# autonomousvision/transfuser

Measured on AMD Instinct MI355X. Metric: training samples/sec (RGB+LiDAR pair), bs=10/GPU, higher is better.
Workload: dtype f32; 1 GPU; TransFuser LidarCenterNet (RegNetY-3.2GF x2, 168.0 M params) full train step, B=10/GPU, 3x256x704 RGB + 3x256x256 BEV, fp32, dropout 0.10, hipGraph replay; global_batch=10, parallelism=dp1, grad_allreduce=none (1 rank), build_id=21d3d8ecc43e0770

## Files before the change

### include/transfuser_hip.h

```cpp
#ifndef TRANSFUSER_HIP_H
#define TRANSFUSER_HIP_H
#include <stdint.h>
#ifdef __cplusplus
extern "C" {
#endif

int tf_version(void);
const char* tf_last_error(void);
const char* tf_build_id(void);
long tf_streamk_launches(void);
int tf_gemm_epi16(int on);
long tf_gemm_epi16_launches(void);

int tf_set_precision(int mode);
int tf_get_precision(void);
int tf_autotune(int enable);
int tf_force_plan(int bm, int bn, int bk, int splitk);
int tf_force_dma(int kind, int splitk);
int tf_plans_count(void);
int tf_plans_clear(void);
int tf_plans_save(const char* path);
int tf_plans_load(const char* path);


// ... 14 lines not shown
int tf_gemm_f32(const tf_gemm_desc* d, void* stream);
long tf_gemm_splitk_ws_floats(const tf_gemm_desc* d);
int tf_gemm_pair_begin(void);
int tf_gemm_pair_end(void* stream);
long tf_gemm_pair_count(int singles);

typedef struct {
    int B, Hi, Wi, Cin, Ho, Wo, Cout, ksize, stride, pad, groups;
} tf_conv_geom;
int tf_conv2d_fwd_f32(const tf_conv_geom* g, const float* x, const float* w, const float* bias, float* y, int relu, void* stream);
int tf_conv2d_fwd_colstat_f32(const tf_conv_geom* g, const float* x, const float* w, const float* bias, float* y, float* colstat, int* colstat_nparts,
                              void* stream);
int tf_conv2d_dgrad_f32(const tf_conv_geom* g, const float* dy, const float* w, float* dx, int accumulate, void* stream);
int tf_conv2d_wgrad_f32(const tf_conv_geom* g, const float* dy, const float* x, float* dw, int accumulate, void* stream);

int tf_conv3x3_small_fwd_f32(const float* x, const float* w, const float* bias, float* y, int B, int H, int W, int Cin, int Cout, int relu, void* stream);
int tf_conv3x3_small_dgrad_f32(const float* dy, const float* w, float* dx, int B, int H, int W, int Cin, int Cout, int accumulate, void* stream);
long tf_conv3x3_small_wgrad_ws_floats(void);
int tf_conv3x3_small_wgrad_f32(const float* dy, const float* x, float* dw, int B, int H, int W, int Cin, int Cout, int accumulate, float* ws, void* stream);

int tf_bn_finalize_parts_f32(const float* parts, int nparts, int rows, int C, const float* gamma, const float* beta, float* running_mean, float* running_var,
                             float momentum, float eps, float* save_mean, float* save_invstd, float* coef_out, void* stream);
int tf_colsum_bnrelu_parts_f32(const float* x, const float* coef, int nseg, int rows_per_seg, int C, float* ws, int* nchunks, void* stream);
int tf_se_excite_fwd_parts_f32(const float* parts, int nchunks, float scale, const float* W1, const float* b1, const float* W2, const float* b2, int B, int C,
                               int Cr, float* s_out, float* g1, float* gate, float* bwd_scratch, void* stream);
int tf_se_scale_bn_fwd_f32(const float* x, const float* coef, const float* gate, float* y, int B, int HW, int C, void* stream);
int tf_se_gate_grad_parts_f32(const float* dy, const float* x, const float* coef, int B, int HW, int C, float* ws, int* nchunks, void* stream);
int tf_se_excite_bwd_parts_f32(const float* parts, int nchunks, const float* gate, const float* s, const float* g1, const float* W1, const float* W2, int B,
                               int C, int Cr, float* dW1, float* db1, float* dW2, float* db2, float* ds, float* scratch, int scratch_is_zero, void* stream);
int tf_bn_bwd_remask_f32(const float* dz, const float* x, const float* fwd_coef, int rows, int C, const float* gamma, const float* save_mean,
                         const float* save_invstd, float* dx, float* dgamma, float* dbeta, float* ws, void* stream);
int tf_bn_bwd_remask_se_f32(const float* dy, const float* gate, const float* dmean, int B, int HW, int C, const float* x, const float* fcoef, const float* gamma,
                            const float* save_mean, const float* save_invstd, float* dx, float* dgamma, float* dbeta, float* ws, void* stream);

int tf_dwconv7_fwd_f32(const float* x, const float* w, const float* bias, float* y, int B, int H, int W, int C, int flip, int accumulate, void* stream);
int tf_dwconv7_wgrad_f32(const float* dy, const float* x, float* dw, float* dbias, int B, int H, int W, int C, void* stream);
int tf_gelu_fwd_f32(const float* x, float* y, int64_t n, void* stream);
int tf_gelu_bwd_f32(const float* dy, const float* x, float* dx, int64_t n, void* stream);
int tf_colscale_add_f32(const float* x, const float* gamma, const float* beta, const float* res, float* y, int64_t rows, int C, void* stream);
int tf_colsum_mul_f32(const float* a, const float* b, int rows, int C, float* out, int accumulate, float* ws, void* stream);
int tf_colsum_multi_f32(int n, const float* const* xs, const int* Cs, const long* lds, float* const* outs, int rows, void* stream);

int tf_cast16_f32(const float* x, int rows, int cols, int ldx, void* y16, int ldy, void* y16t, int ldyt, int dtype, void* stream);
typedef struct { const float* x; void* y16; void* y16t; int rows, cols, ldx, ldy, ldyt, tile0; } tf_cast16_item;
int tf_cast16_multi_f32(const tf_cast16_item* items_dev, int n_items, int total_tiles, int dtype, void* stream);
int tf_bn_apply16_f32(const float* x, const float* coef, const float* res, int relu, float* y32, int rows, int C, void* y16, void* y16t, int ldyt, int dtype, void* stream);
int tf_se_scale_bn16_f32(const float* x, const float* coef, const float* gate, int B, int HW, int C, void* y16, void* y16t, int ldyt, int dtype, void* stream);
int tf_bn_bwd16_f32(const float* dz, const float* z, const float* x, int rows, int C, const float* gamma, const float* save_mean, const float* save_invstd, float* dx32,
                    float* dres, float* dgamma, float* dbeta, float* ws, void* dx16, void* dx16t, int ldyt, int dtype, void* stream);
int tf_bn_bwd_remask16_f32(const float* dz, const float* x, const float* fcoef, int rows, int C, const float* gamma, const float* save_mean, const float* save_invstd,
                           float* dx32, float* dgamma, float* dbeta, float* ws, void* dx16, void* dx16t, int ldyt, int dtype, void* stream);
int tf_layernorm_fwd16_f32(const float* x, const float* gamma, const float* beta, void* y16, int ldy, void* y16t, int ldyt, float* mean, float* rstd,
                           int rows, int C, float eps, int dtype, void* stream);
int tf_gemm16_nt_f32(const void* a16, const void* b16, float* c, int m, int n, int k, int lda, int ldb, int ldc, const float* bias, const float* res, int ldres,
                     float alpha, int relu, int accumulate, const float* mask, int ldmask, int dtype, void* stream);
int tf_gemm16_nt_colstat_f32(const void* a16, const void* b16, float* c, int m, int n, int k, int lda, int ldb, int ldc, int dtype, float* colstat,
                             int* colstat_nparts, void* stream);
int tf_add_strided2_f32(const float* src, float* dst, int B, int Ho, int Wo, int C, int Hi, int Wi, void* stream);
int tf_im2col3x3_f32(const float* x, float* cols, int B, int H, int W, int C, void* stream);

int tf_conv3x3_thin_supported(int Cin, int Cout);
int tf_conv3x3_thin_fwd_f32(const float* x, const float* w, const float* bias, float* y, int B, int H, int W, int Cin, int Cout, void* stream);
int tf_conv3x3_thin_dgrad_f32(const float* dy, const float* w, const float* relu_mask, float* dx, int B, int H, int W, int Cin, int Cout, int accumulate,
                              void* stream);
long tf_conv3x3_thin_wgrad_ws_floats(void);
int tf_conv3x3_thin_wgrad_f32(const float* dy, const float* x, float* dw, float* dbias, int B, int H, int W, int Cin, int Cout, int accumulate, float* ws,
// ... 171 lines not shown
```

### transfuser_amd/csrc/reduce.cpp

```cpp
#include <cstdlib>
#include "tf_common.h"
#include "../../include/transfuser_hip.h"

using namespace tf;

namespace {

template <int V> struct vecf { float v[V]; };
template <int V> __device__ __forceinline__ vecf<V> ldv(const float* p) {
    vecf<V> r;
    if (V == 4) { float4 t = *reinterpret_cast<const float4*>(p); r.v[0] = t.x; r.v[1 % V] = t.y; r.v[2 % V] = t.z; r.v[3 % V] = t.w; }
    else r.v[0] = *p;
    return r;
}
template <int V> __device__ __forceinline__ void stv(float* p, const vecf<V>& a) {
    if (V == 4) *reinterpret_cast<float4*>(p) = make_float4(a.v[0], a.v[1 % V], a.v[2 % V], a.v[3 % V]);
    else *p = a.v[0];
}

constexpr int kBnSlots = 16;
constexpr int kMaxChunks = 512;
constexpr long kWsFloats = 4L << 20;
constexpr int kTickets = 4096;

// ... 78 lines not shown
template <int V> struct BnReluMulF {
    const float* dy; const float* x; const float* coef; int C;
    __device__ __forceinline__ void eval(long row, int c, vecf<V>* o) const {
        vecf<V> g = ldv<V>(dy + row * C + c), a = ldv<V>(x + row * C + c), sc = ldv<V>(coef + c), sh = ldv<V>(coef + C + c);
#pragma unroll
        for (int i = 0; i < V; ++i) o[0].v[i] = g.v[i] * fmaxf(a.v[i] * sc.v[i] + sh.v[i], 0.f);
    }
};
template <int V> struct BnBwdRemaskF {
    const float* dz; const float* x; const float* coef; const float* mean; const float* invstd; int C;
    __device__ __forceinline__ void eval(long row, int c, vecf<V>* o) const {
        vecf<V> g = ldv<V>(dz + row * C + c), a = ldv<V>(x + row * C + c), m = ldv<V>(mean + c), s = ldv<V>(invstd + c), sc = ldv<V>(coef + c), sh = ldv<V>(coef + C + c);
#pragma unroll
        for (int i = 0; i < V; ++i) {
            if (!(a.v[i] * sc.v[i] + sh.v[i] > 0.f)) g.v[i] = 0.f;
            o[0].v[i] = g.v[i];
            o[1].v[i] = g.v[i] * ((a.v[i] - m.v[i]) * s.v[i]);
        }
    }
};

template <int V> struct SeBnBwdRemaskF {
    const float* dy; const float* gate; const float* dmean; const float* x; const float* coef; const float* mean; const float* invstd; int C; int HW; float inv_hw;
    __device__ __forceinline__ void eval(long row, int c, vecf<V>* o) const {
        const long bc = (row / HW) * C + c;
        vecf<V> g = ldv<V>(dy + row * C + c), a = ldv<V>(x + row * C + c), m = ldv<V>(mean + c), s = ldv<V>(invstd + c), sc = ldv<V>(coef + c), sh = ldv<V>(coef + C + c);
        vecf<V> gt = ldv<V>(gate + bc), dm = ldv<V>(dmean + bc);
#pragma unroll
        for (int i = 0; i < V; ++i) {
            float gi = g.v[i] * (1.f / (1.f + expf(-gt.v[i]))) + dm.v[i] * inv_hw;
            if (!(a.v[i] * sc.v[i] + sh.v[i] > 0.f)) gi = 0.f;
            o[0].v[i] = gi;
            o[1].v[i] = gi * ((a.v[i] - m.v[i]) * s.v[i]);
        }
    }
};

template <int V, int NACC, class F>
__global__ void __launch_bounds__(256) colreduce_kernel(F f, int rows_per_seg, int C, int CTV, int rows_per_chunk, float* __restrict__ ws, int atomic,
                                                        float scale) {
    __shared__ __attribute__((aligned(16))) float red[NACC][256][V];
    const int tid = threadIdx.x;
    const int rpp = 256 / CTV;
    const int cq = tid % CTV, rl = tid / CTV;
    const int c = (blockIdx.x * CTV + cq) * V;
    const int seg = blockIdx.z, chunk = blockIdx.y;
    const int r0 = chunk * rows_per_chunk;
    int r1 = r0 + rows_per_chunk;
    if (r1 > rows_per_seg) r1 = rows_per_seg;
    vecf<V> acc[NACC];
#pragma unroll
    for (int a = 0; a < NACC; ++a)
#pragma unroll
        for (int i = 0; i < V; ++i) acc[a].v[i] = 0.f;
    if (rl < rpp) {
        const long base = (long)seg * rows_per_seg;
        int r = r0 + rl;
        if (atomic >= 0)
            for (; r < r1; r += 4 * rpp) {
                vecf<V> o[4][NACC];
#pragma unroll
                for (int u = 0; u < 4; ++u) {
                    const int rr = r + u * rpp;
                    f.eval(base + (rr < r1 ? rr : r1 - 1), c, o[u]);
                }
#pragma unroll
// ... 171 lines not shown
    coef[c] = sc;
    coef[C + c] = beta[c] - mean * sc;
    if (rmean) {
        rmean[c] = (1.f - momentum) * rmean[c] + momentum * mean;
        const float unb = (n > 1.f) ? var * (n / (n - 1.f)) : var;
        rvar[c] = (1.f - momentum) * rvar[c] + momentum * unb;
    }
}
__global__ void bn_eval_coef_kernel(const float* __restrict__ gamma, const float* __restrict__ beta, const float* __restrict__ rmean,
                                    const float* __restrict__ rvar, float* __restrict__ coef, int C, float eps) {
    const int c = blockIdx.x * 256 + threadIdx.x;
    if (c >= C) return;
    const float sc = gamma[c] / sqrtf(rvar[c] + eps);
    coef[c] = sc;
    coef[C + c] = beta[c] - rmean[c] * sc;
}
__global__ void __launch_bounds__(256) bn_bwd_finalize_kernel(const float* __restrict__ ws, const float* __restrict__ gamma, const float* __restrict__ mean,
                                                              const float* __restrict__ invstd, float* __restrict__ dgamma, float* __restrict__ dbeta,
                                                              float* __restrict__ coef, int C, int nch, float n) {
    const int c0 = blockIdx.x * 4 + (threadIdx.x >> 6), lane = threadIdx.x & 63;
    const bool live = c0 < C;
    const int c = live ? c0 : 0;
    float sg, sgx;
    chunk_sum2(ws + c, ws + C + c, 2L * C, nch, lane, live, sg, sgx);
    if (!live || lane != 0) return;
    if (dgamma) dgamma[c] += sgx;
    if (dbeta) dbeta[c] += sg;
    const float A = gamma[c] * invstd[c];
    const float Bc = -A * invstd[c] * (sgx / n);
    coef[c] = A;
    coef[C + c] = Bc;
    coef[2 * C + c] = -A * (sg / n) - Bc * mean[c];
}
__global__ void __launch_bounds__(256) se_bwd_finalize_kernel(const float* __restrict__ ws, const float* __restrict__ gate, float* __restrict__ dgate, int C,
                                                              int nch, int nseg) {
    const int i = blockIdx.x * 4 + (threadIdx.x >> 6), lane = threadIdx.x & 63;
    const bool live = i < nseg * C;
    const int seg = live ? i / C : 0, c = live ? i - seg * C : 0;
    const float s = chunk_sum(ws + (long)seg * nch * C + c, C, nch, lane, live);
    if (live && lane == 0) {
        const float sg = 1.f / (1.f + expf(-gate[i]));
        dgate[i] = s * sg * (1.f - sg);
    }
}

template <int V>
__global__ void __launch_bounds__(256) bn_apply_kernel(const float* __restrict__ x, const float* __restrict__ coef, const float* __restrict__ res,
                                                       float* __restrict__ y, long nvec, int C, int relu) {
    const int cv = C / V;
    for (long i = (long)blockIdx.x * 256 + threadIdx.x; i < nvec; i += (long)gridDim.x * 256) {
        const int c = (int)(i % cv) * V;
        vecf<V> a = ldv<V>(x + i * V), s = ldv<V>(coef + c), t = ldv<V>(coef + C + c);
        vecf<V> r;
        if (res) r = ldv<V>(res + i * V);
#pragma unroll
        for (int k = 0; k < V; ++k) {
            float v = a.v[k] * s.v[k] + t.v[k];
            if (res) v += r.v[k];
            if (relu) v = fmaxf(v, 0.f);
            a.v[k] = v;
        }
        stv<V>(y + i * V, a);
    }
}
template <int V>
__global__ void __launch_bounds__(256) bn_bwd_apply_kernel(const float* __restrict__ dz, const float* __restrict__ z, const float* __restrict__ x,
// ... 507 lines not shown
    const bool v4 = (C % 4 == 0) && aligned16(dz) && aligned16(x) && aligned16(dx) && aligned16(fcoef);
    RedPlan p = plan_reduce(rows, C, 1, 2, v4);
    BnBwdRemaskF<4> f4{dz, x, fcoef, save_mean, save_invstd, C};
    BnBwdRemaskF<1> f1{dz, x, fcoef, save_mean, save_invstd, C};
    launch_reduce<2>(p, f4, f1, rows, C, 1, ws, stream);
    TF_LAUNCH(bn_bwd_finalize_kernel, dim3(cdiv(C, 4)), dim3(256), stream, (const float*)ws, gamma, save_mean, save_invstd, dgamma, dbeta, coef, C, p.nchunks,
              (float)rows);
    const long n = (long)rows * C;
    if (v4) TF_LAUNCH(bn_bwd_apply_remask_kernel<4>, dim3(ew_blocks(n / 4)), dim3(256), stream, dz, x, fcoef, (const float*)coef, dx, n / 4, C);
    else TF_LAUNCH(bn_bwd_apply_remask_kernel<1>, dim3(ew_blocks(n)), dim3(256), stream, dz, x, fcoef, (const float*)coef, dx, n, C);
    return launch_status("tf_bn_bwd_remask_f32");
}

extern "C" int tf_bn_bwd_remask_se_f32(const float* dy, const float* gate, const float* dmean, int B, int HW, int C, const float* x, const float* fcoef,
                                       const float* gamma, const float* save_mean, const float* save_invstd, float* dx, float* dgamma, float* dbeta, float* ws,
                                       void* stream) {
    TF_REQUIRE(dy && gate && dmean && x && fcoef && gamma && save_mean && save_invstd && dx && ws && B > 0 && HW > 0 && C > 0, "tf_bn_bwd_remask_se_f32: bad arguments");
    const int rows = B * HW;
    float* coef = ws + kWsFloats / 2;
    const bool v4 = (C % 4 == 0) && aligned16(dy) && aligned16(x) && aligned16(dx) && aligned16(fcoef) && aligned16(gate) && aligned16(dmean);
    RedPlan p = plan_reduce(rows, C, 1, 2, v4);
    const float inv_hw = 1.f / (float)HW;
    SeBnBwdRemaskF<4> f4{dy, gate, dmean, x, fcoef, save_mean, save_invstd, C, HW, inv_hw};
    SeBnBwdRemaskF<1> f1{dy, gate, dmean, x, fcoef, save_mean, save_invstd, C, HW, inv_hw};
    launch_reduce<2>(p, f4, f1, rows, C, 1, ws, stream);
    TF_LAUNCH(bn_bwd_finalize_kernel, dim3(cdiv(C, 4)), dim3(256), stream, (const float*)ws, gamma, save_mean, save_invstd, dgamma, dbeta, coef, C, p.nchunks,
              (float)rows);
    const long n = (long)rows * C;
    if (v4) TF_LAUNCH(bn_bwd_apply_remask_se_kernel<4>, dim3(ew_blocks(n / 4)), dim3(256), stream, dy, gate, dmean, x, fcoef, (const float*)coef, dx, n / 4, C, (long)HW * C / 4, inv_hw);
    else TF_LAUNCH(bn_bwd_apply_remask_se_kernel<1>, dim3(ew_blocks(n)), dim3(256), stream, dy, gate, dmean, x, fcoef, (const float*)coef, dx, n, C, (long)HW * C, inv_hw);
    return launch_status("tf_bn_bwd_remask_se_f32");
}

extern "C" int tf_colsum_mul_f32(const float* a, const float* b, int rows, int C, float* out, int accumulate, float* ws, void* stream) {
    TF_REQUIRE(a && b && out && ws && rows > 0 && C > 0, "tf_colsum_mul_f32: bad arguments");
    RedPlan p = plan_reduce(rows, C, 1, 1, aligned16(a) && aligned16(b));
    MulF<4> f4{a, b, C};
    MulF<1> f1{a, b, C};
    launch_reduce<1>(p, f4, f1, rows, C, 1, ws, stream);
    TF_LAUNCH(colsum_finalize_kernel, dim3(cdiv((long)C, 4)), dim3(256), stream, (const float*)ws, out, C, p.nchunks, 1, 1.f, accumulate);
    return launch_status("tf_colsum_mul_f32");
}

extern "C" int tf_colsum_multi_f32(int n, const float* const* xs, const int* Cs, const long* lds, float* const* outs, int rows, void* stream) {
    TF_REQUIRE(n >= 1 && n <= kMultiMax && xs && Cs && lds && outs && rows > 0, "tf_colsum_multi_f32: 1 <= n <= %d matrices with rows > 0", kMultiMax);
    MultiSum d;
    d.n = n;
    int strips = 0;
    for (int i = 0; i < kMultiMax; ++i) {
        const int j = i < n ? i : n - 1;
        d.x[i] = xs[j]; d.out[i] = outs[j]; d.C[i] = Cs[j]; d.ld[i] = lds[j];
        d.strip0[i] = strips;
        if (i < n) {
            TF_REQUIRE(xs[i] && outs[i] && Cs[i] > 0 && Cs[i] % 4 == 0 && lds[i] % 4 == 0 && lds[i] >= Cs[i] && aligned16(xs[i]),
                       "tf_colsum_multi_f32: entry %d needs C %% 4 == 0, ld %% 4 == 0, ld >= C and a 16-byte aligned base", i);
            strips += cdiv(Cs[i], 32);
        }
    }
    d.strip0[kMultiMax] = strips;
    TF_LAUNCH(colsum_multi_kernel, dim3(strips), dim3(256), stream, d, rows);
    return launch_status("tf_colsum_multi_f32");
}

extern "C" int tf_bn_apply16_f32(const float* x, const float* coef, const float* res, int relu, float* y32, int rows, int C, void* y16, void* y16t, int ldyt,
                                 int dtype, void* stream) {
    TF_REQUIRE(x && coef && tile16_ok(rows, C, y16, y16t, ldyt, dtype) && aligned16(x) && aligned16(coef) && (!res || aligned16(res)) && (!y32 || aligned16(y32)),
// ... 44 lines not shown
```

### transfuser_amd/csrc/se.cpp

```cpp
#include "tf_common.h"
#include "../../include/transfuser_hip.h"

using namespace tf;

namespace {

constexpr int SE_MAXB = 16;
constexpr int SE_SPLIT = 8;
constexpr int SE_U = 4;
constexpr int SE_MAXC = 3072, SE_MAXR = 1024;

__device__ __forceinline__ float dot4(const float4 a, const float4 b) { return a.x * b.x + a.y * b.y + a.z * b.z + a.w * b.w; }

template <int U, int NK>
__device__ __forceinline__ void se_dots(const float* const* w, const float* __restrict__ vec, int n4, int lane, float* acc) {
    float4 wv[U][NK];
#pragma unroll
    for (int i = 0; i < NK; ++i) {
        const int k4 = lane + 64 * i, kc = k4 < n4 ? k4 : n4 - 1;
#pragma unroll
        for (int u = 0; u < U; ++u) wv[u][i] = reinterpret_cast<const float4*>(w[u])[kc];
    }
#pragma unroll
    for (int i = 0; i < NK; ++i) {
// ... 97 lines not shown
            }
        }
        __syncthreads();
        for (int nb = n0 + wave * SE_U; nb < n1; nb += nw * SE_U) {
            float acc[SE_U];
            const float* w[SE_U];
#pragma unroll
            for (int u = 0; u < SE_U; ++u) {
                acc[u] = 0.f;
                w[u] = W2 + (long)((nb + u < n1) ? nb + u : n1 - 1) * Cr;
            }
            for (int j = lane; j < Cr; j += 64) {
#pragma unroll
                for (int u = 0; u < SE_U; ++u) acc[u] += w[u][j] * hh[j];
            }
#pragma unroll
            for (int u = 0; u < SE_U; ++u) {
                const float a = wave_sum(acc[u]);
                if (lane == 0 && nb + u < n1) store2(nb + u, a);
            }
        }
    }
}

__global__ void __launch_bounds__(256) se_zero_kernel(float* __restrict__ p, int n) {
    const int i = blockIdx.x * 256 + threadIdx.x;
    if (i < n) p[i] = 0.f;
}

constexpr int SE_ROWS = 8;
__global__ void __launch_bounds__(256) se_excite_bwd2_kernel(const float* __restrict__ dgate, const float* __restrict__ g1, const float* __restrict__ W2,
                                                             int B, int C, int Cr, float* __restrict__ dW2, float* __restrict__ db2,
                                                             float* __restrict__ dg1, float* __restrict__ ds_zero, int nch = 0,
                                                             const float* __restrict__ gate = nullptr) {
    __shared__ float dgs[SE_MAXB][SE_ROWS];
    for (long i = (long)blockIdx.x * 256 + threadIdx.x; i < (long)B * C; i += (long)gridDim.x * 256) ds_zero[i] = 0.f;
    __shared__ float g1s[SE_MAXB * SE_MAXR / 2];
    const int n0 = blockIdx.x * SE_ROWS, tid = threadIdx.x;
    const int rows = (C - n0 < SE_ROWS) ? C - n0 : SE_ROWS;
    for (int i = tid; i < B * SE_ROWS; i += 256) {
        const int b = i / SE_ROWS, r = i % SE_ROWS;
        float v = 0.f;
        if (r < rows) {
            if (nch > 0) {
                const float* p = dgate + (long)b * nch * C + n0 + r;
                float v1 = 0.f, v2 = 0.f, v3 = 0.f;
                int j = 0;
                for (; j + 3 < nch; j += 4) { v += p[(long)j * C]; v1 += p[(long)(j + 1) * C]; v2 += p[(long)(j + 2) * C]; v3 += p[(long)(j + 3) * C]; }
                for (; j < nch; ++j) v += p[(long)j * C];
                v = (v + v1) + (v2 + v3);
                const float sg = 1.f / (1.f + expf(-gate[(long)b * C + n0 + r]));
                v *= sg * (1.f - sg);
            } else {
                v = dgate[(long)b * C + n0 + r];
            }
        }
        dgs[b][r] = v;
    }
    for (int i = tid; i < B * Cr; i += 256) g1s[i] = g1[i];
    __syncthreads();
    for (int i = tid; i < rows * Cr; i += 256) {
        const int r = i / Cr, j = i - r * Cr;
        float v = 0.f;
        for (int b = 0; b < B; ++b) v += dgs[b][r] * g1s[b * Cr + j];
        dW2[(long)(n0 + r) * Cr + j] += v;
    }
    if (tid < rows && db2) {
        float v = 0.f;
        for (int b = 0; b < B; ++b) v += dgs[b][tid];
        db2[n0 + tid] += v;
    }
    for (int j = tid; j < Cr; j += 256) {
        float acc[SE_MAXB];
#pragma unroll
        for (int b = 0; b < SE_MAXB; ++b) acc[b] = 0.f;
        float wv[SE_ROWS];
#pragma unroll
        for (int r = 0; r < SE_ROWS; ++r) wv[r] = W2[(long)(n0 + (r < rows ? r : rows - 1)) * Cr + j];
#pragma unroll
        for (int r = 0; r < SE_ROWS; ++r) {
            const float w = r < rows ? wv[r] : 0.f;
#pragma unroll
// ... 80 lines not shown
    return launch_status("tf_se_excite_fwd_f32");
}

extern "C" int tf_se_excite_bwd_f32(const float* dgate, const float* s, const float* g1, const float* W1, const float* W2, int B, int C, int Cr,
                                    float* dW1, float* db1, float* dW2, float* db2, float* ds, float* scratch, int scratch_is_zero, void* stream) {
    TF_REQUIRE(dgate && s && g1 && W1 && W2 && dW1 && dW2 && ds && scratch && B > 0 && B <= SE_MAXB && C > 0 && Cr > 0 &&
                   (long)B * Cr <= SE_MAXB * SE_MAXR / 2, "tf_se_excite_bwd_f32: bad arguments (B <= 16, B*Cr <= 8192)");
    if (!scratch_is_zero) TF_LAUNCH(se_zero_kernel, dim3(cdiv((long)B * Cr, 256)), dim3(256), stream, scratch, B * Cr);
    TF_LAUNCH(se_excite_bwd2_kernel, dim3(cdiv(C, SE_ROWS)), dim3(256), stream, dgate, g1, W2, B, C, Cr, dW2, db2, scratch, ds);
    TF_LAUNCH(se_excite_bwd1_kernel, dim3(cdiv(C, 32), SE_JS), dim3(256), stream, (const float*)scratch, g1, s, W1, B, C, Cr, dW1, db1, ds);
    return launch_status("tf_se_excite_bwd_f32");
}

extern "C" int tf_se_excite_fwd_parts_f32(const float* parts, int nchunks, float scale, const float* W1, const float* b1, const float* W2, const float* b2, int B,
                                          int C, int Cr, float* s_out, float* g1, float* gate, float* bwd_scratch, void* stream) {
    TF_REQUIRE(parts && nchunks > 0 && W1 && W2 && s_out && g1 && gate && B > 0 && C > 0 && Cr > 0 && C <= SE_MAXC && Cr <= SE_MAXR,
               "tf_se_excite_fwd_parts_f32: bad arguments (C <= 3072, Cr <= 1024)");
    const bool v4 = C % 4 == 0 && Cr % 4 == 0 && aligned16(W1) && aligned16(W2);
    if (v4) TF_LAUNCH(se_excite_fwd_kernel<true>, dim3(B, SE_SPLIT), dim3(1024), stream, parts, W1, b1, W2, b2, C, Cr, g1, gate, bwd_scratch, nchunks, scale, s_out);
    else TF_LAUNCH(se_excite_fwd_kernel<false>, dim3(B, SE_SPLIT), dim3(1024), stream, parts, W1, b1, W2, b2, C, Cr, g1, gate, bwd_scratch, nchunks, scale, s_out);
    return launch_status("tf_se_excite_fwd_parts_f32");
}

extern "C" int tf_se_excite_bwd_parts_f32(const float* parts, int nchunks, const float* gate, const float* s, const float* g1, const float* W1, const float* W2,
                                          int B, int C, int Cr, float* dW1, float* db1, float* dW2, float* db2, float* ds, float* scratch, int scratch_is_zero,
                                          void* stream) {
    TF_REQUIRE(parts && nchunks > 0 && gate && s && g1 && W1 && W2 && dW1 && dW2 && ds && scratch && B > 0 && B <= SE_MAXB && C > 0 && Cr > 0 &&
                   (long)B * Cr <= SE_MAXB * SE_MAXR / 2, "tf_se_excite_bwd_parts_f32: bad arguments (B <= 16, B*Cr <= 8192)");
    if (!scratch_is_zero) TF_LAUNCH(se_zero_kernel, dim3(cdiv((long)B * Cr, 256)), dim3(256), stream, scratch, B * Cr);
    TF_LAUNCH(se_excite_bwd2_kernel, dim3(cdiv(C, SE_ROWS)), dim3(256), stream, parts, g1, W2, B, C, Cr, dW2, db2, scratch, ds, nchunks, gate);
    TF_LAUNCH(se_excite_bwd1_kernel, dim3(cdiv(C, 32), SE_JS), dim3(256), stream, (const float*)scratch, g1, s, W1, B, C, Cr, dW1, db1, ds);
    return launch_status("tf_se_excite_bwd_parts_f32");
}
```

### transfuser_amd/functions.py

```python
import math

import torch

from . import ops


_INPLACE = False
_collect = None


class inplace_param_grads:
    def __enter__(self):
        global _INPLACE
        self.prev, _INPLACE = _INPLACE, True

    def __exit__(self, *a):
        global _INPLACE
        _INPLACE = self.prev


def gbuf(p):
    if _collect is not None:
        t = _collect.get(id(p))
        if t is None:
# ... 390 lines not shown
            out, o16, o16t = ops.bn_apply16(y3, coef3, sc, True)
            st3 = (sm3, si3)
            out._lp16 = (out._version, o16, o16t)
        else:
            out, st3 = _bn(y3, bn3, res=sc, relu=True, stat=cs3)
        ctx.saved = (x, blk, y1, z1, st1, y2, z2, st2, s, g1, gate, z2ss, y3, st3, yd, std, out, x2s, (lp, x16t, z16t))
        return out

    @staticmethod
    def backward(ctx, dout):
        if ctx.saved is None:
            raise RuntimeError("YBlockFn: trying to backward through the graph a second time: the saved activations are freed by the first backward "
                               "(retain_graph is not supported by the block Functions)")
        x, blk, y1, z1, st1, y2, z2, st2, s, g1, gate, z2ss, y3, st3, yd, std, out, x2s, (lp, x16t, z16t) = ctx.saved
        B, H, W, Cin = x.shape
        _, Ho, Wo, C = out.shape
        x2 = x.view(-1, Cin)
        w3 = blk.conv3.conv.weight
        if lp:
            bn3 = blk.conv3.bn
            if len(st3) == 2:
                _, d16, d16t, dsc = ops.bn_bwd16(dout.contiguous(), out, y3, bn3.weight, st3[0], st3[1], gbuf(bn3.weight), gbuf(bn3.bias), want_dres=True)
            else:
                dy3, dsc = _bn_bwd(dout.contiguous(), out, y3, bn3, st3, want_dres=True)
                d16, d16t = ops.cast16(dy3.view(-1, C))
            dz2s = _c1x1_bwd16(d16, d16t, z16t, w2d(w3), w2d(gbuf(w3))).view(B, Ho, Wo, C)
        else:
            dy3, dsc = _bn_bwd(dout.contiguous(), out, y3, blk.conv3.bn, st3, want_dres=True)
            dy3_2 = dy3.view(-1, C)
            dz2s = _c1x1_bwd(dy3_2, z2ss, w2d(w3), w2d(gbuf(w3))).view(B, Ho, Wo, C)
        se = blk.se
        if z2 is None:
            ds = ops.se_gate_excite_bn_bwd(dz2s, y2, st2[2], gate, s, g1, se.fc1.weight, se.fc2.weight, gbuf(se.fc1.weight), gbuf(se.fc1.bias),
                                           gbuf(se.fc2.weight), gbuf(se.fc2.bias))
            bn2 = blk.conv2.bn
            if ops.FUSE_SE_BN_BWD:
                dy2 = ops.bn_bwd_remask_se(dz2s, gate, ds, y2, st2[2], bn2.weight, st2[0], st2[1], gbuf(bn2.weight), gbuf(bn2.bias))
            else:
                dz2 = ops.se_scale_bwd_x(dz2s, gate, ds, y2.shape)
                dy2 = ops.bn_bwd_remask(dz2, y2, st2[2], bn2.weight, st2[0], st2[1], gbuf(bn2.weight), gbuf(bn2.bias))
        else:
            dgate = ops.se_scale_bwd_gate(dz2s, z2, gate)
            if B <= 16 and C <= ops.SE_FUSED_MAX_C and B * g1.shape[1] <= 8192:
                ds = ops.se_excite_bwd(dgate, s, g1, se.fc1.weight, se.fc2.weight, gbuf(se.fc1.weight), gbuf(se.fc1.bias), gbuf(se.fc2.weight),
                                       gbuf(se.fc2.bias))
            else:
                ops.linear_wgrad(dgate, g1, w2d(gbuf(se.fc2.weight)))
                bias_grad(dgate, se.fc2.bias)
                dg1 = ops.linear_dgrad(dgate, w2d(se.fc2.weight))
                dg1 = ops.relu_mask(dg1, g1, out=dg1)
                ops.linear_wgrad(dg1, s, w2d(gbuf(se.fc1.weight)))
                bias_grad(dg1, se.fc1.bias)
                ds = ops.linear_dgrad(dg1, w2d(se.fc1.weight))
            dz2 = ops.se_scale_bwd_x(dz2s, gate, ds, z2.shape)
            dy2, _ = _bn_bwd(dz2, z2, y2, blk.conv2.bn, st2)
        w2 = blk.conv2.conv.weight
        if z1 is None:
            bn1 = blk.conv1.bn
            ops.grouped_bnrelu_wgrad(dy2, y1, st1[2], gbuf(w2), stride=blk.stride)
            dz1 = ops.conv_dgrad(dy2, w2, y1.shape, blk.stride, 1, blk.groups)
            if lp:
                _, e16, e16t = ops.bn_bwd_remask16(dz1, y1, st1[2], bn1.weight, st1[0], st1[1], gbuf(bn1.weight), gbuf(bn1.bias))
            else:
                dy1 = ops.bn_bwd_remask(dz1, y1, st1[2], bn1.weight, st1[0], st1[1], gbuf(bn1.weight), gbuf(bn1.bias))
        else:
            ops.conv_wgrad(dy2, z1, gbuf(w2), blk.stride, 1, blk.groups)
            dz1 = ops.conv_dgrad(dy2, w2, z1.shape, blk.stride, 1, blk.groups)
# ... 672 lines not shown
```

### transfuser_amd/ops.py

```python
import ctypes

import os
import sys

import torch

from . import _lib
from ._lib import ConvGeom, GemmDesc, c_p, check, ptr, stream_of

byref = ctypes.byref

_ws_cache = {}


def L():
    return _lib.load()


def workspace(device):
    key = (str(device), torch.cuda.current_stream(device).cuda_stream if getattr(device, "type", str(device)[:4]) == "cuda" else 0)
    ws = _ws_cache.get(key)
    if ws is None:
        L().tf_workspace_bytes.restype = ctypes.c_long
        ws = torch.zeros(L().tf_workspace_bytes() // 4, dtype=torch.float32, device=device)
# ... 944 lines not shown
                  "tf_conv3x3_grouped_s2_wgrad_f32")
            _census_end(_e, "conv wgrad g2", (B, H, W, C, C, 3, 2, C // 24), 2.0 * dy.shape[0] * dy.shape[1] * dy.shape[2] * C * 24 * 9)
            return
        check(L().tf_conv3x3_grouped_bnrelu_wgrad_f32(ptr(_c(dy)), ptr(_c(x)), ptr(coef), wptr(dw), B, H, W, C, int(accumulate), ptr(_grouped_ws(x.device)),
                                                      stream_of(dy)), "tf_conv3x3_grouped_bnrelu_wgrad_f32")
        _census_end(_e, "conv wgrad g", (B, H, W, C, C, 3, 1, C // 24), 2.0 * B * H * W * C * 24 * 9)
    run()
    return dw


def se_squeeze_excite_bn_fwd(y, coef, w1, b1, w2, b2):
    B, H, W, C = y.shape
    Cr = w1.shape[0]
    nch = ctypes.c_int(0)
    ws = workspace(y.device)
    check(L().tf_colsum_bnrelu_parts_f32(ptr(_c(y)), ptr(coef), B, H * W, C, ptr(ws), byref(nch), stream_of(y)), "tf_colsum_bnrelu_parts_f32")
    s = torch.empty(B, C, dtype=torch.float32, device=y.device)
    buf = torch.empty(2, B, Cr, dtype=torch.float32, device=y.device)
    g1 = buf[0]
    g1._bwd_scratch = buf[1]
    gate = torch.empty(B, C, dtype=torch.float32, device=y.device)
    check(L().tf_se_excite_fwd_parts_f32(ptr(ws), nch.value, ctypes.c_float(1.0 / (H * W)), wptr(w1), ptr(b1), wptr(w2), ptr(b2), B, C, Cr, ptr(s), ptr(g1),
                                         ptr(gate), ptr(buf[1]), stream_of(y)), "tf_se_excite_fwd_parts_f32")
    return s, g1, gate


def se_scale_bn_fwd(y, coef, gate):
    B, H, W, C = y.shape
    out = torch.empty_like(y)
    check(L().tf_se_scale_bn_fwd_f32(ptr(_c(y)), ptr(coef), ptr(_c(gate)), ptr(out), B, H * W, C, stream_of(y)), "tf_se_scale_bn_fwd_f32")
    return out


def se_gate_excite_bn_bwd(dz2s, y, coef, gate, s, g1, w1, w2, dw1, db1, dw2, db2):
    B, H, W, C = y.shape
    Cr = w1.shape[0]
    nch = ctypes.c_int(0)
    ws = workspace(y.device)
    check(L().tf_se_gate_grad_parts_f32(ptr(_c(dz2s)), ptr(_c(y)), ptr(coef), B, H * W, C, ptr(ws), byref(nch), stream_of(y)), "tf_se_gate_grad_parts_f32")
    ds = torch.empty(B, C, dtype=torch.float32, device=y.device)
    scratch = getattr(g1, "_bwd_scratch", None)
    zeroed = scratch is not None
    if zeroed:
        g1._bwd_scratch = None
    else:
        scratch = torch.empty(B, Cr, dtype=torch.float32, device=y.device)
    check(L().tf_se_excite_bwd_parts_f32(ptr(ws), nch.value, ptr(_c(gate)), ptr(_c(s)), ptr(_c(g1)), wptr(w1), wptr(w2), B, C, Cr, wptr(dw1), ptr(db1), wptr(dw2),
                                         ptr(db2), ptr(ds), ptr(scratch), int(zeroed), stream_of(y)), "tf_se_excite_bwd_parts_f32")
    return ds


def bn_bwd_remask(dz, x, coef, gamma, sm, si, dgamma, dbeta):
    C = x.shape[-1]
    rows = x.numel() // C
    dx = torch.empty_like(x)
    check(L().tf_bn_bwd_remask_f32(ptr(_c(dz)), ptr(_c(x)), ptr(coef), rows, C, ptr(gamma), ptr(sm), ptr(si), ptr(dx), ptr(dgamma), ptr(dbeta),
                                   ptr(workspace(x.device)), stream_of(x)), "tf_bn_bwd_remask_f32")
    return dx


FUSE_SE_BN_BWD = os.environ.get("TF_FUSE_SE_BN_BWD", "1") != "0"


def bn_bwd_remask_se(dy, gate, dmean, x, coef, gamma, sm, si, dgamma, dbeta):
    B, H, W, C = x.shape
    dx = torch.empty_like(x)
    _h = _hbm_begin()
    check(L().tf_bn_bwd_remask_se_f32(ptr(_c(dy)), ptr(gate), ptr(_c(dmean)), B, H * W, C, ptr(_c(x)), ptr(coef), ptr(gamma), ptr(sm), ptr(si), ptr(dx), ptr(dgamma),
                                      ptr(dbeta), ptr(workspace(x.device)), stream_of(x)), "tf_bn_bwd_remask_se_f32")
    _hbm_end(_h, "batchnorm backward (reduce + finalize + apply)", 4 * x.numel() * 5)
    return dx


def bn_bwd(dz, z, x, gamma, sm, si, dgamma, dbeta, want_dres=False):
    C = x.shape[-1]
    rows = x.numel() // C
    dx = torch.empty_like(x)
    dres = torch.empty_like(x) if want_dres else None
    zacc = zero_scratch(32 * C, x.device) if not _DBG_LEGACY_BNB else None
    _h = _hbm_begin()
    check(L().tf_bn_bwd_f32(ptr(_c(dz)), ptr(z), ptr(_c(x)), rows, C, ptr(gamma), ptr(sm), ptr(si), ptr(dx), ptr(dres), ptr(dgamma), ptr(dbeta),
                            ptr(workspace(x.device)), ptr(zacc), stream_of(x)), "tf_bn_bwd_f32")
    _hbm_end(_h, "batchnorm backward (reduce + finalize + apply)", 4 * x.numel() * ((2 + (z is not None)) * 2 + 1 + (dres is not None)))
    return dx, dres


FUSE_DROPOUT = os.environ.get("TF_FUSE_DROPOUT", "1") != "0"
LN_FWD16 = os.environ.get("TF_LN_FWD16", "1") != "0"


COLSUM_MULTI = os.environ.get("TF_COLSUM_MULTI", "1") != "0"


def colsum_multi(pairs):
    rows = pairs[0][0].shape[0]
    ok = 1 <= len(pairs) <= 8 and all(x.dim() == 2 and x.shape[0] == rows and x.stride(1) == 1 and x.shape[1] % 4 == 0 and x.stride(0) % 4 == 0 and
                                      x.data_ptr() % 16 == 0 and o.is_contiguous() and o.numel() == x.shape[1] for x, o in pairs)
    if not ok:
        for x, o in pairs:
            colsum(x.contiguous(), 1, rows, x.shape[1], 1.0, out=o.view(1, -1), accumulate=True)
# ... 508 lines not shown
```

Baseline: 230.7 samples/s.

## Fuse SE gate-grad and BN-backward reductions into one five-output pass

In the SE block backward, the gate-gradient reduction and the batchnorm backward reduction used to read dy and x in two separate full passes. A single per-(batch, chunk) pass now computes five partial sums: the gate grad term, masked dy, masked dy*xhat, the mask count and masked xhat. Because the SE gradient term is constant per (b, c), the BN sums can be rebuilt algebraically from these partials in a small finalize kernel, so the second full reduction over the activations goes away. In exchange the parts buffer is larger, the finalize does more work, and results are cached on the ds tensor and matched by a pointer/version key.

Result: no change. 232.6 samples/s (median of 6 runs) (+0.8%).

```diff
diff --git a/include/transfuser_hip.h b/include/transfuser_hip.h
--- a/include/transfuser_hip.h
+++ b/include/transfuser_hip.h
@@ -70,6 +70,13 @@
                          const float* save_invstd, float* dx, float* dgamma, float* dbeta, float* ws, void* stream);
 int tf_bn_bwd_remask_se_f32(const float* dy, const float* gate, const float* dmean, int B, int HW, int C, const float* x, const float* fcoef, const float* gamma,
                             const float* save_mean, const float* save_invstd, float* dx, float* dgamma, float* dbeta, float* ws, void* stream);
+int tf_se_bn_bwd_parts_f32(const float* dy, const float* x, const float* fcoef, const float* save_mean, const float* save_invstd, int B, int HW, int C,
+                           float* parts, int* nchunks, void* stream);
+int tf_se_excite_bwd_parts5_f32(const float* parts, int nchunks, const float* gate, const float* s, const float* g1, const float* W1, const float* W2, int B,
+                                int C, int Cr, float* dW1, float* db1, float* dW2, float* db2, float* ds, float* scratch, int scratch_is_zero, void* stream);
+int tf_bn_bwd_remask_se_parts_f32(const float* dy, const float* gate, const float* dmean, const float* parts, int nchunks, int B, int HW, int C, const float* x,
+                                  const float* fcoef, const float* gamma, const float* save_mean, const float* save_invstd, float* dx, float* dgamma,
+                                  float* dbeta, float* ws, void* stream);
 
 int tf_dwconv7_fwd_f32(const float* x, const float* w, const float* bias, float* y, int B, int H, int W, int C, int flip, int accumulate, void* stream);
 int tf_dwconv7_wgrad_f32(const float* dy, const float* x, float* dw, float* dbias, int B, int H, int W, int C, void* stream);
diff --git a/transfuser_amd/csrc/reduce.cpp b/transfuser_amd/csrc/reduce.cpp
--- a/transfuser_amd/csrc/reduce.cpp
+++ b/transfuser_amd/csrc/reduce.cpp
@@ -134,6 +134,23 @@
             if (!(a.v[i] * sc.v[i] + sh.v[i] > 0.f)) gi = 0.f;
             o[0].v[i] = gi;
             o[1].v[i] = gi * ((a.v[i] - m.v[i]) * s.v[i]);
+        }
+    }
+};
+
+template <int V> struct SeBnPartsF {
+    const float* dy; const float* x; const float* coef; const float* mean; const float* invstd; int C;
+    __device__ __forceinline__ void eval(long row, int c, vecf<V>* o) const {
+        vecf<V> g = ldv<V>(dy + row * C + c), a = ldv<V>(x + row * C + c), m = ldv<V>(mean + c), s = ldv<V>(invstd + c), sc = ldv<V>(coef + c), sh = ldv<V>(coef + C + c);
+#pragma unroll
+        for (int i = 0; i < V; ++i) {
+            const bool on = a.v[i] * sc.v[i] + sh.v[i] > 0.f;
+            const float xh = (a.v[i] - m.v[i]) * s.v[i], gm = on ? g.v[i] : 0.f;
+            o[0].v[i] = g.v[i] * fmaxf(a.v[i] * sc.v[i] + sh.v[i], 0.f);
+            o[1].v[i] = gm;
+            o[2].v[i] = gm * xh;
+            o[3].v[i] = on ? 1.f : 0.f;
+            o[4].v[i] = on ? xh : 0.f;
         }
     }
 };
@@ -371,6 +388,47 @@
     coef[C + c] = Bc;
     coef[2 * C + c] = -A * (sg / n) - Bc * mean[c];
 }
+__global__ void __launch_bounds__(256) bn_bwd_finalize_se_kernel(const float* __restrict__ parts, const float* __restrict__ gate, const float* __restrict__ dmean,
+                                                                 const float* __restrict__ gamma, const float* __restrict__ mean,
+                                                                 const float* __restrict__ invstd, float* __restrict__ dgamma, float* __restrict__ dbeta,
+                                                                 float* __restrict__ coef, int B, int C, int nch, float inv_hw, float n) {
+    const int c0 = blockIdx.x * 4 + (threadIdx.x >> 6), lane = threadIdx.x & 63;
+    const bool live = c0 < C;
+    const int c = live ? c0 : 0;
+    const int items = B * nch;
+    float sg = 0.f, sgx = 0.f;
+    if (live)
+        for (int j = lane; j < items; j += 128) {
+            float p[2][4], gt[2], dm[2];
+#pragma unroll
+            for (int u = 0; u < 2; ++u) {
+                const int jj = j + 64 * u, jc = jj < items ? jj : items - 1;
+                const float* q = parts + ((long)jc * 5 + 1) * C + c;
+                const long bc = (long)(jc / nch) * C + c;
+#pragma unroll
+                for (int k = 0; k < 4; ++k) p[u][k] = q[(long)k * C];
+                gt[u] = gate[bc]; dm[u] = dmean[bc];
+            }
+#pragma unroll
+            for (int u = 0; u < 2; ++u) {
+                const bool in = j + 64 * u < items;
+                const float s = 1.f / (1.f + expf(-gt[u])), t = dm[u] * inv_hw;
+                const float vg = s * p[u][0] + t * p[u][2], vgx = s * p[u][1] + t * p[u][3];
+                sg += in ? vg : 0.f;
+                sgx += in ? vgx : 0.f;
+            }
+        }
+    sg = wave_sum(sg);
+    sgx = wave_sum(sgx);
+    if (!live || lane != 0) return;
+    if (dgamma) dgamma[c] += sgx;
+    if (dbeta) dbeta[c] += sg;
+    const float A = gamma[c] * invstd[c];
+    const float Bc = -A * invstd[c] * (sgx / n);
+    coef[c] = A;
+    coef[C + c] = Bc;
+    coef[2 * C + c] = -A * (sg / n) - Bc * mean[c];
+}
 __global__ void __launch_bounds__(256) se_bwd_finalize_kernel(const float* __restrict__ ws, const float* __restrict__ gate, float* __restrict__ dgate, int C,
                                                               int nch, int nseg) {
     const int i = blockIdx.x * 4 + (threadIdx.x >> 6), lane = threadIdx.x & 63;
@@ -944,6 +1002,34 @@
     return launch_status("tf_bn_bwd_remask_se_f32");
 }
 
+extern "C" int tf_se_bn_bwd_parts_f32(const float* dy, const float* x, const float* fcoef, const float* save_mean, const float* save_invstd, int B, int HW,
+                                      int C, float* parts, int* nchunks, void* stream) {
+    TF_REQUIRE(dy && x && fcoef && save_mean && save_invstd && parts && nchunks && B > 0 && HW > 0 && C > 0, "tf_se_bn_bwd_parts_f32: bad arguments");
+    RedPlan p = plan_reduce(HW, C, B, 5, aligned16(x) && aligned16(fcoef) && aligned16(dy) && aligned16(save_mean) && aligned16(save_invstd) && aligned16(parts));
+    cap_chunks(p, HW, 8);
+    SeBnPartsF<4> f4{dy, x, fcoef, save_mean, save_invstd, C};
+    SeBnPartsF<1> f1{dy, x, fcoef, save_mean, save_invstd, C};
+    launch_reduce<5>(p, f4, f1, HW, C, B, parts, stream);
+    *nchunks = p.nchunks;
+    return launch_status("tf_se_bn_bwd_parts_f32");
+}
+extern "C" int tf_bn_bwd_remask_se_parts_f32(const float* dy, const float* gate, const float* dmean, const float* parts, int nchunks, int B, int HW, int C,
+                                             const float* x, const float* fcoef, const float* gamma, const float* save_mean, const float* save_invstd, float* dx,
+                                             float* dgamma, float* dbeta, float* ws, void* stream) {
+    TF_REQUIRE(dy && gate && dmean && parts && nchunks > 0 && nchunks <= 8 && x && fcoef && gamma && save_mean && save_invstd && dx && ws && B > 0 && HW > 0 && C > 0,
+               "tf_bn_bwd_remask_se_parts_f32: bad arguments (1 <= nchunks <= 8)");
+    const int rows = B * HW;
+    float* coef = ws + kWsFloats / 2;
+    const bool v4 = (C % 4 == 0) && aligned16(dy) && aligned16(x) && aligned16(dx) && aligned16(fcoef) && aligned16(gate) && aligned16(dmean);
+    const float inv_hw = 1.f / (float)HW;
+    TF_LAUNCH(bn_bwd_finalize_se_kernel, dim3(cdiv(C, 4)), dim3(256), stream, parts, gate, dmean, gamma, save_mean, save_invstd, dgamma, dbeta, coef, B, C, nchunks,
+              inv_hw, (float)rows);
+    const long n = (long)rows * C;
+    if (v4) TF_LAUNCH(bn_bwd_apply_remask_se_kernel<4>, dim3(ew_blocks(n / 4)), dim3(256), stream, dy, gate, dmean, x, fcoef, (const float*)coef, dx, n / 4, C, (long)HW * C / 4, inv_hw);
+    else TF_LAUNCH(bn_bwd_apply_remask_se_kernel<1>, dim3(ew_blocks(n)), dim3(256), stream, dy, gate, dmean, x, fcoef, (const float*)coef, dx, n, C, (long)HW * C, inv_hw);
+    return launch_status("tf_bn_bwd_remask_se_parts_f32");
+}
+
 extern "C" int tf_colsum_mul_f32(const float* a, const float* b, int rows, int C, float* out, int accumulate, float* ws, void* stream) {
     TF_REQUIRE(a && b && out && ws && rows > 0 && C > 0, "tf_colsum_mul_f32: bad arguments");
     RedPlan p = plan_reduce(rows, C, 1, 1, aligned16(a) && aligned16(b));
diff --git a/transfuser_amd/csrc/se.cpp b/transfuser_amd/csrc/se.cpp
--- a/transfuser_amd/csrc/se.cpp
+++ b/transfuser_amd/csrc/se.cpp
@@ -153,7 +153,7 @@
 __global__ void __launch_bounds__(256) se_excite_bwd2_kernel(const float* __restrict__ dgate, const float* __restrict__ g1, const float* __restrict__ W2,
                                                              int B, int C, int Cr, float* __restrict__ dW2, float* __restrict__ db2,
                                                              float* __restrict__ dg1, float* __restrict__ ds_zero, int nch = 0,
-                                                             const float* __restrict__ gate = nullptr) {
+                                                             const float* __restrict__ gate = nullptr, long cstride = 0) {
     __shared__ float dgs[SE_MAXB][SE_ROWS];
     for (long i = (long)blockIdx.x * 256 + threadIdx.x; i < (long)B * C; i += (long)gridDim.x * 256) ds_zero[i] = 0.f;
     __shared__ float g1s[SE_MAXB * SE_MAXR / 2];
@@ -164,11 +164,12 @@
         float v = 0.f;
         if (r < rows) {
             if (nch > 0) {
-                const float* p = dgate + (long)b * nch * C + n0 + r;
+                const long cs = cstride > 0 ? cstride : C;
+                const float* p = dgate + (long)b * nch * cs + n0 + r;
                 float v1 = 0.f, v2 = 0.f, v3 = 0.f;
                 int j = 0;
-                for (; j + 3 < nch; j += 4) { v += p[(long)j * C]; v1 += p[(long)(j + 1) * C]; v2 += p[(long)(j + 2) * C]; v3 += p[(long)(j + 3) * C]; }
-                for (; j < nch; ++j) v += p[(long)j * C];
+                for (; j + 3 < nch; j += 4) { v += p[(long)j * cs]; v1 += p[(long)(j + 1) * cs]; v2 += p[(long)(j + 2) * cs]; v3 += p[(long)(j + 3) * cs]; }
+                for (; j < nch; ++j) v += p[(long)j * cs];
                 v = (v + v1) + (v2 + v3);
                 const float sg = 1.f / (1.f + expf(-gate[(long)b * C + n0 + r]));
                 v *= sg * (1.f - sg);
@@ -315,3 +316,14 @@
     TF_LAUNCH(se_excite_bwd1_kernel, dim3(cdiv(C, 32), SE_JS), dim3(256), stream, (const float*)scratch, g1, s, W1, B, C, Cr, dW1, db1, ds);
     return launch_status("tf_se_excite_bwd_parts_f32");
 }
+
+extern "C" int tf_se_excite_bwd_parts5_f32(const float* parts, int nchunks, const float* gate, const float* s, const float* g1, const float* W1, const float* W2,
+                                           int B, int C, int Cr, float* dW1, float* db1, float* dW2, float* db2, float* ds, float* scratch, int scratch_is_zero,
+                                           void* stream) {
+    TF_REQUIRE(parts && nchunks > 0 && gate && s && g1 && W1 && W2 && dW1 && dW2 && ds && scratch && B > 0 && B <= SE_MAXB && C > 0 && Cr > 0 &&
+                   (long)B * Cr <= SE_MAXB * SE_MAXR / 2, "tf_se_excite_bwd_parts5_f32: bad arguments (B <= 16, B*Cr <= 8192)");
+    if (!scratch_is_zero) TF_LAUNCH(se_zero_kernel, dim3(cdiv((long)B * Cr, 256)), dim3(256), stream, scratch, B * Cr);
+    TF_LAUNCH(se_excite_bwd2_kernel, dim3(cdiv(C, SE_ROWS)), dim3(256), stream, parts, g1, W2, B, C, Cr, dW2, db2, scratch, ds, nchunks, gate, 5L * C);
+    TF_LAUNCH(se_excite_bwd1_kernel, dim3(cdiv(C, 32), SE_JS), dim3(256), stream, (const float*)scratch, g1, s, W1, B, C, Cr, dW1, db1, ds);
+    return launch_status("tf_se_excite_bwd_parts5_f32");
+}
diff --git a/transfuser_amd/functions.py b/transfuser_amd/functions.py
--- a/transfuser_amd/functions.py
+++ b/transfuser_amd/functions.py
@@ -446,7 +446,7 @@
         se = blk.se
         if z2 is None:
             ds = ops.se_gate_excite_bn_bwd(dz2s, y2, st2[2], gate, s, g1, se.fc1.weight, se.fc2.weight, gbuf(se.fc1.weight), gbuf(se.fc1.bias),
-                                           gbuf(se.fc2.weight), gbuf(se.fc2.bias))
+                                           gbuf(se.fc2.weight), gbuf(se.fc2.bias), stats=(st2[0], st2[1]))
             bn2 = blk.conv2.bn
             if ops.FUSE_SE_BN_BWD:
                 dy2 = ops.bn_bwd_remask_se(dz2s, gate, ds, y2, st2[2], bn2.weight, st2[0], st2[1], gbuf(bn2.weight), gbuf(bn2.bias))
diff --git a/transfuser_amd/ops.py b/transfuser_amd/ops.py
--- a/transfuser_amd/ops.py
+++ b/transfuser_amd/ops.py
@@ -1000,12 +1000,17 @@
     return out
 
 
-def se_gate_excite_bn_bwd(dz2s, y, coef, gate, s, g1, w1, w2, dw1, db1, dw2, db2):
+SE_BN_BWD_PARTS = os.environ.get("TF_SE_BN_PARTS", "1") != "0"
+
+
+def _se_bn_parts_key(dy, x, coef):
+    return (dy.data_ptr(), dy._version, x.data_ptr(), x._version, coef.data_ptr(), tuple(x.shape))
+
+
+def se_gate_excite_bn_bwd(dz2s, y, coef, gate, s, g1, w1, w2, dw1, db1, dw2, db2, stats=None):
     B, H, W, C = y.shape
     Cr = w1.shape[0]
     nch = ctypes.c_int(0)
-    ws = workspace(y.device)
-    check(L().tf_se_gate_grad_parts_f32(ptr(_c(dz2s)), ptr(_c(y)), ptr(coef), B, H * W, C, ptr(ws), byref(nch), stream_of(y)), "tf_se_gate_grad_parts_f32")
     ds = torch.empty(B, C, dtype=torch.float32, device=y.device)
     scratch = getattr(g1, "_bwd_scratch", None)
     zeroed = scratch is not None
@@ -1013,6 +1018,16 @@
         g1._bwd_scratch = None
     else:
         scratch = torch.empty(B, Cr, dtype=torch.float32, device=y.device)
+    if stats is not None and FUSE_SE_BN_BWD and SE_BN_BWD_PARTS and L().tf_get_precision() in (0, 2):
+        parts = torch.empty(B * 8 * 5 * C, dtype=torch.float32, device=y.device)
+        check(L().tf_se_bn_bwd_parts_f32(ptr(_c(dz2s)), ptr(_c(y)), ptr(coef), ptr(stats[0]), ptr(stats[1]), B, H * W, C, ptr(parts), byref(nch), stream_of(y)),
+              "tf_se_bn_bwd_parts_f32")
+        check(L().tf_se_excite_bwd_parts5_f32(ptr(parts), nch.value, ptr(_c(gate)), ptr(_c(s)), ptr(_c(g1)), wptr(w1), wptr(w2), B, C, Cr, wptr(dw1), ptr(db1),
+                                              wptr(dw2), ptr(db2), ptr(ds), ptr(scratch), int(zeroed), stream_of(y)), "tf_se_excite_bwd_parts5_f32")
+        ds._se_bn_parts = (parts, nch.value, _se_bn_parts_key(dz2s, y, coef))
+        return ds
+    ws = workspace(y.device)
+    check(L().tf_se_gate_grad_parts_f32(ptr(_c(dz2s)), ptr(_c(y)), ptr(coef), B, H * W, C, ptr(ws), byref(nch), stream_of(y)), "tf_se_gate_grad_parts_f32")
     check(L().tf_se_excite_bwd_parts_f32(ptr(ws), nch.value, ptr(_c(gate)), ptr(_c(s)), ptr(_c(g1)), wptr(w1), wptr(w2), B, C, Cr, wptr(dw1), ptr(db1), wptr(dw2),
                                          ptr(db2), ptr(ds), ptr(scratch), int(zeroed), stream_of(y)), "tf_se_excite_bwd_parts_f32")
     return ds
@@ -1033,7 +1048,14 @@
 def bn_bwd_remask_se(dy, gate, dmean, x, coef, gamma, sm, si, dgamma, dbeta):
     B, H, W, C = x.shape
     dx = torch.empty_like(x)
+    parts = getattr(dmean, "_se_bn_parts", None)
     _h = _hbm_begin()
+    if parts is not None and parts[2] == _se_bn_parts_key(dy, x, coef):
+        check(L().tf_bn_bwd_remask_se_parts_f32(ptr(_c(dy)), ptr(gate), ptr(_c(dmean)), ptr(parts[0]), parts[1], B, H * W, C, ptr(_c(x)), ptr(coef), ptr(gamma),
+                                                ptr(sm), ptr(si), ptr(dx), ptr(dgamma), ptr(dbeta), ptr(workspace(x.device)), stream_of(x)),
+              "tf_bn_bwd_remask_se_parts_f32")
+        _hbm_end(_h, "batchnorm backward (reduce + finalize + apply)", 4 * x.numel() * 3)
+        return dx
     check(L().tf_bn_bwd_remask_se_f32(ptr(_c(dy)), ptr(gate), ptr(_c(dmean)), B, H * W, C, ptr(_c(x)), ptr(coef), ptr(gamma), ptr(sm), ptr(si), ptr(dx), ptr(dgamma),
                                       ptr(dbeta), ptr(workspace(x.device)), stream_of(x)), "tf_bn_bwd_remask_se_f32")
     _hbm_end(_h, "batchnorm backward (reduce + finalize + apply)", 4 * x.numel() * 5)
```
